# suous/RecNeXt

Measured on AMD Instinct MI355X. Metric: images/sec RecNeXt-M3 224x224 bf16, higher is better.
Workload: dtype bf16

## Files before the change

### recnext_amd/csrc/rcx_mlp.hip

```cpp
#include "rcx_common.h"
#include "rcx_launch.h"
#include "rcx_gelu.h"

namespace rcx {
namespace mlp {

typedef float f32x16 __attribute__((ext_vector_type(16)));
typedef float f32x4q __attribute__((ext_vector_type(4)));
typedef float f32x2q __attribute__((ext_vector_type(2)));
typedef __bf16 bf16x8 __attribute__((ext_vector_type(8)));
typedef __bf16 bf16x4 __attribute__((ext_vector_type(4)));
typedef unsigned u32x4q __attribute__((ext_vector_type(4)));
typedef unsigned u32x2q __attribute__((ext_vector_type(2)));

__device__ __forceinline__ void wave_sync()
{
    __builtin_amdgcn_fence(__ATOMIC_RELEASE, "wavefront");
    __builtin_amdgcn_wave_barrier();
    __builtin_amdgcn_fence(__ATOMIC_ACQUIRE, "wavefront");
}

template <int KS1, int CT, int RD>
__device__ __forceinline__ void hidden_tile_ring(const u32x4q* Lc, const float* b1t, int lane, int h, const bf16x8 (&zb)[KS1], f32x16 (&d2)[CT])
{
    constexpr int R1 = KS1 < RD ? KS1 : RD, N2 = 2 * CT, R2 = N2 < RD ? N2 : RD;
    u32x4q ring[RD];
#pragma unroll
    for (int j = 0; j < R1; ++j) ring[j] = Lc[j * 64 + lane];
    f32x16 d1;
#pragma unroll
    for (int i = 0; i < 16; ++i) d1[i] = 0.f;
#pragma unroll
    for (int ks = 0; ks < KS1; ++ks) {
        const bf16x8 a = __builtin_bit_cast(bf16x8, ring[ks % R1]);
        if (ks + R1 < KS1) ring[ks % R1] = Lc[(ks + R1) * 64 + lane];
        d1 = __builtin_amdgcn_mfma_f32_32x32x16_bf16(a, zb[ks], d1, 0, 0, 0);
    }
#pragma unroll
    for (int f = 0; f < R2; ++f) ring[f] = Lc[(KS1 + 2 * (f % CT) + f / CT) * 64 + lane];
    bf16x8 hb[2];
    gelu_f32x2 gv[8];
#pragma unroll
    for (int g = 0; g < 4; ++g) {
        const f32x4q bb = *reinterpret_cast<const f32x4q*>(b1t + 8 * g + 4 * h);
        gv[2 * g] = gelu_f32x2{d1[4 * g] + bb.x, d1[4 * g + 1] + bb.y};
        gv[2 * g + 1] = gelu_f32x2{d1[4 * g + 2] + bb.z, d1[4 * g + 3] + bb.w};
    }
    {
        gelu_f32x2 ga[4] = {gv[0], gv[1], gv[2], gv[3]}, gb[4] = {gv[4], gv[5], gv[6], gv[7]};
        gelu2x_batch<4>(ga);
        gelu2x_batch<4>(gb);
#pragma unroll
        for (int i = 0; i < 4; ++i) { gv[i] = ga[i]; gv[4 + i] = gb[i]; }
    }
#pragma unroll
    for (int g = 0; g < 4; ++g) {
        hb[g >> 1][4 * (g & 1) + 0] = (__bf16)gv[2 * g].x; hb[g >> 1][4 * (g & 1) + 1] = (__bf16)gv[2 * g].y;
        hb[g >> 1][4 * (g & 1) + 2] = (__bf16)gv[2 * g + 1].x; hb[g >> 1][4 * (g & 1) + 3] = (__bf16)gv[2 * g + 1].y;
    }
#pragma unroll
    for (int f = 0; f < N2; ++f) {
        const bf16x8 a = __builtin_bit_cast(bf16x8, ring[f % R2]);
        if (f + R2 < N2) ring[f % R2] = Lc[(KS1 + 2 * ((f + R2) % CT) + (f + R2) / CT) * 64 + lane];
        d2[f % CT] = __builtin_amdgcn_mfma_f32_32x32x16_bf16(a, hb[f / CT], d2[f % CT], 0, 0, 0);
    }
}


template <int KS1, int HT, int CT, int NW, int WPS, bool KX, bool OX, bool STAGED>
__global__ void __launch_bounds__(64 * NW, WPS)
k_channel_mlp(const bf16_t* __restrict__ z, const bf16_t* __restrict__ xres, bf16_t* __restrict__ y, const u32x4q* __restrict__ wfrag, const float* __restrict__ bias,
              int M, int C, int ntiles)
{
    extern __shared__ __attribute__((aligned(16))) unsigned char lds_raw[];
    constexpr int NF = HT * KS1 + CT * 2 * HT;
    const u32x4q* const Lf = reinterpret_cast<const u32x4q*>(lds_raw);
    const float* const Lb1 = reinterpret_cast<const float*>(lds_raw + (size_t)NF * 1024);
    const float* const Lb2 = Lb1 + 32 * HT;
    {
        u32x4q* Lw = reinterpret_cast<u32x4q*>(lds_raw);
        for (int i = threadIdx.x; i < NF * 64; i += 64 * NW) Lw[i] = wfrag[i];
        float* Lb = reinterpret_cast<float*>(lds_raw + (size_t)NF * 1024);
        for (int i = threadIdx.x; i < 32 * (HT + CT); i += 64 * NW) Lb[i] = bias[i];
    }
    __syncthreads();
    const int wave = threadIdx.x >> 6, lane = threadIdx.x & 63, r = lane & 31, h = lane >> 5;
    const unsigned nbytes = (unsigned)M * (unsigned)C * 2u;
    const __amdgpu_buffer_rsrc_t zsrc = __builtin_amdgcn_make_buffer_rsrc((void*)z, 0, nbytes, 0x00020000);
    const __amdgpu_buffer_rsrc_t xsrc = __builtin_amdgcn_make_buffer_rsrc((void*)xres, 0, nbytes, 0x00020000);
    const __amdgpu_buffer_rsrc_t ysrc = __builtin_amdgcn_make_buffer_rsrc((void*)y, 0, nbytes, 0x00020000);
    unsigned zk[KS1], oc[CT][4];
#pragma unroll
    for (int ks = 0; ks < KS1; ++ks) zk[ks] = KX || 16 * ks + 8 * h < C ? 2u * (16 * ks + 8 * h) : 0x80000000u;
#pragma unroll
    for (int ct = 0; ct < CT; ++ct)
#pragma unroll
        for (int g = 0; g < 4; ++g) oc[ct][g] = OX || 32 * ct + 8 * g + 4 * h < C ? 2u * (32 * ct + 8 * g + 4 * h) : 0x80000000u;

    auto hidden_tile = [&](int ht, const bf16x8 (&zb)[KS1], f32x16 (&d2)[CT]) {
        hidden_tile_ring<KS1, CT, 4>(Lf + (size_t)ht * (KS1 + 2 * CT) * 64, Lb1 + 32 * ht, lane, h, zb, d2);
    };
    const int stride = gridDim.x * NW;
    int tile = blockIdx.x * NW + wave;
    if constexpr (STAGED) {
        constexpr int ZP = 32 * KS1 + 16, OP = 128 * CT + 16;
        constexpr int WREG = 32 * (ZP > OP ? ZP : OP);
        unsigned char* const Lt = lds_raw + (size_t)NF * 1024 + sizeof(float) * 32 * (HT + CT) + (size_t)wave * WREG;
        const unsigned RB = 2u * (unsigned)C;
        unsigned go[KS1], za[KS1], oa[KS1];
        bool live[KS1];
#pragma unroll
        for (int i = 0; i < KS1; ++i) {
            const unsigned o = 1024u * i + 16u * lane, t = o / RB, bb = o - t * RB;
            live[i] = o < 32u * RB;
            go[i] = live[i] ? o : 0x80000000u;
            za[i] = t * ZP + bb;
            oa[i] = t * OP + 2u * bb;
        }
        u32x4q zq[KS1];
        auto load_z = [&](int t) {
#pragma unroll
            for (int i = 0; i < KS1; ++i) zq[i] = __builtin_bit_cast(u32x4q, __builtin_amdgcn_raw_buffer_load_b128(zsrc, (int)((unsigned)t * 32u * RB + go[i]), 0, 0));
        };
        if (tile < ntiles) load_z(tile);
        for (; tile < ntiles; tile += stride) {
            const unsigned base = (unsigned)tile * 32u * RB;
#pragma unroll
            for (int i = 0; i < KS1; ++i)
                if (live[i]) *reinterpret_cast<u32x4q*>(Lt + za[i]) = zq[i];
            wave_sync();
            bf16x8 zb[KS1];
#pragma unroll
            for (int ks = 0; ks < KS1; ++ks) {
                u32x4q v = *reinterpret_cast<const u32x4q*>(Lt + r * ZP + 32 * ks + 16 * h);
                if (!KX && ks == KS1 - 1 && !(16 * ks + 8 * h < C)) v = u32x4q{0u, 0u, 0u, 0u};
                zb[ks] = __builtin_bit_cast(bf16x8, v);
            }
            wave_sync();
            if (tile + stride < ntiles) load_z(tile + stride);
            u32x4q xq[KS1];
#pragma unroll
            for (int i = 0; i < KS1; ++i) xq[i] = __builtin_bit_cast(u32x4q, __builtin_amdgcn_raw_buffer_load_b128(xsrc, (int)(base + go[i]), 0, 0));
            f32x16 d2[CT];
#pragma unroll
            for (int ct = 0; ct < CT; ++ct)
#pragma unroll
                for (int i = 0; i < 16; ++i) d2[ct][i] = 0.f;
#pragma unroll 1
            for (int ht = 0; ht < HT; ++ht) hidden_tile(ht, zb, d2);
#pragma unroll
            for (int ct = 0; ct < CT; ++ct)
#pragma unroll
                for (int g = 0; g < 4; ++g) {
                    const f32x4q bb = *reinterpret_cast<const f32x4q*>(Lb2 + 32 * ct + 8 * g + 4 * h);
                    *reinterpret_cast<f32x4q*>(Lt + r * OP + 4 * (32 * ct + 8 * g + 4 * h)) =
                        f32x4q{d2[ct][4 * g] + bb.x, d2[ct][4 * g + 1] + bb.y, d2[ct][4 * g + 2] + bb.z, d2[ct][4 * g + 3] + bb.w};
                }
            wave_sync();
#pragma unroll
            for (int i = 0; i < KS1; ++i) {
                if (!live[i]) continue;
                const f32x4q lo = *reinterpret_cast<const f32x4q*>(Lt + oa[i]), hi = *reinterpret_cast<const f32x4q*>(Lt + oa[i] + 16);
                const u32x4q xv = xq[i];
                bf16x8 o;
                o[0] = (__bf16)(lo.x + __uint_as_float(xv.x << 16)); o[1] = (__bf16)(lo.y + __uint_as_float(xv.x & 0xffff0000u));
                o[2] = (__bf16)(lo.z + __uint_as_float(xv.y << 16)); o[3] = (__bf16)(lo.w + __uint_as_float(xv.y & 0xffff0000u));
                o[4] = (__bf16)(hi.x + __uint_as_float(xv.z << 16)); o[5] = (__bf16)(hi.y + __uint_as_float(xv.z & 0xffff0000u));
                o[6] = (__bf16)(hi.z + __uint_as_float(xv.w << 16)); o[7] = (__bf16)(hi.w + __uint_as_float(xv.w & 0xffff0000u));
                __builtin_amdgcn_raw_buffer_store_b128(__builtin_bit_cast(u32x4q, o), ysrc, (int)(base + go[i]), 0, 0);
            }
            wave_sync();
        }
        return;
    }
    u32x4q zf[KS1];
    auto load_z = [&](int t) {
        const unsigned row = (unsigned)(32 * t + r) * (unsigned)C * 2u;
#pragma unroll
        for (int ks = 0; ks < KS1; ++ks) zf[ks] = __builtin_bit_cast(u32x4q, __builtin_amdgcn_raw_buffer_load_b128(zsrc, (int)(row + zk[ks]), 0, 0));
    };
    if (tile < ntiles) load_z(tile);
    for (; tile < ntiles; tile += stride) {
        const unsigned row = (unsigned)(32 * tile + r) * (unsigned)C * 2u;
        bf16x8 zb[KS1];
#pragma unroll
        for (int ks = 0; ks < KS1; ++ks) zb[ks] = __builtin_bit_cast(bf16x8, zf[ks]);
        if (tile + stride < ntiles) load_z(tile + stride);
        f32x16 d2[CT];
#pragma unroll
        for (int ct = 0; ct < CT; ++ct)
#pragma unroll
            for (int i = 0; i < 16; ++i) d2[ct][i] = 0.f;
#pragma unroll 1
        for (int ht = 0; ht < HT; ++ht) hidden_tile(ht, zb, d2);
        u32x2q xr[CT][4];
#pragma unroll
        for (int ct = 0; ct < CT; ++ct)
#pragma unroll
            for (int g = 0; g < 4; ++g) xr[ct][g] = __builtin_bit_cast(u32x2q, __builtin_amdgcn_raw_buffer_load_b64(xsrc, (int)(row + oc[ct][g]), 0, 0));
#pragma unroll
        for (int ct = 0; ct < CT; ++ct)
#pragma unroll
            for (int g = 0; g < 4; ++g) {
                const f32x4q bb = *reinterpret_cast<const f32x4q*>(Lb2 + 32 * ct + 8 * g + 4 * h);
                const unsigned x0 = xr[ct][g].x, x1 = xr[ct][g].y;
                bf16x4 o;
                o[0] = (__bf16)(d2[ct][4 * g + 0] + bb.x + __uint_as_float(x0 << 16));
                o[1] = (__bf16)(d2[ct][4 * g + 1] + bb.y + __uint_as_float(x0 & 0xffff0000u));
                o[2] = (__bf16)(d2[ct][4 * g + 2] + bb.z + __uint_as_float(x1 << 16));
                o[3] = (__bf16)(d2[ct][4 * g + 3] + bb.w + __uint_as_float(x1 & 0xffff0000u));
                __builtin_amdgcn_raw_buffer_store_b64(__builtin_bit_cast(u32x2q, o), ysrc, (int)(row + oc[ct][g]), 0, 0);
            }
    }
}


template <int KS1, int HT, int CT, int NW, int WPS, int ZH, bool ZPF>
__global__ void __launch_bounds__(64 * NW, WPS)
k_channel_mlp_stream(const bf16_t* __restrict__ z, const bf16_t* __restrict__ xres, bf16_t* __restrict__ y, const u32x4q* __restrict__ wfrag, const float* __restrict__ bias,
                     int M, int C, int nblocks)
{
    extern __shared__ __attribute__((aligned(16))) unsigned char lds_raw[];
    constexpr int NCH = KS1 + 2 * CT, NT = 64 * NW, PER = (NCH * 64 + NT - 1) / NT;
    constexpr bool RAG = NCH * 64 % NT != 0;
    u32x4q* const Lring = reinterpret_cast<u32x4q*>(lds_raw);
    float* const Lb1 = reinterpret_cast<float*>(lds_raw + (size_t)2 * NCH * 1024);
    float* const Lb2 = Lb1 + 32 * HT;
    for (int i = threadIdx.x; i < 32 * (HT + CT); i += NT) Lb1[i] = bias[i];
    const int wave = threadIdx.x >> 6, lane = threadIdx.x & 63, r = lane & 31, h = lane >> 5;
    const unsigned nbytes = (unsigned)M * (unsigned)C * 2u;
    const __amdgpu_buffer_rsrc_t zsrc = __builtin_amdgcn_make_buffer_rsrc((void*)z, 0, nbytes, 0x00020000);
    const __amdgpu_buffer_rsrc_t xsrc = __builtin_amdgcn_make_buffer_rsrc((void*)xres, 0, nbytes, 0x00020000);
    const __amdgpu_buffer_rsrc_t ysrc = __builtin_amdgcn_make_buffer_rsrc((void*)y, 0, nbytes, 0x00020000);
    static_assert(HT % 2 == 0, "the ring alternates two register sets");
    u32x4q cp[2][PER];
    auto request = [&](u32x4q (&dst)[PER], int chunk) {
#pragma unroll
        for (int i = 0; i < PER; ++i)
            if (!RAG || i + 1 < PER || threadIdx.x + i * NT < NCH * 64) dst[i] = wfrag[(size_t)chunk * NCH * 64 + threadIdx.x + i * NT];
    };
    auto deposit = [&](const u32x4q (&src)[PER], int slot) {
        u32x4q* const Ln = Lring + slot * NCH * 64;
#pragma unroll
        for (int i = 0; i < PER; ++i)
            if (!RAG || i + 1 < PER || threadIdx.x + i * NT < NCH * 64) Ln[threadIdx.x + i * NT] = src[i];
    };
    request(cp[0], 0);
    deposit(cp[0], 0);
    request(cp[1], 1 % HT);
    __syncthreads();
    static_assert(CT % 2 == 0, "output in halves of two tiles");
    static_assert(KS1 % ZH == 0, "column parts of whole k-steps");
    constexpr int RB = 32 * KS1, RBH = RB / ZH, KH = KS1 / ZH, ZP = RBH + 16, OP = 256 + 16, IMG = 32 * (ZP > OP ? ZP : OP), NH = CT / 2;
    unsigned char* const Lt = lds_raw + (size_t)2 * NCH * 1024 + sizeof(float) * 32 * (HT + CT) + (size_t)wave * IMG;
    unsigned zo[KS1], za[KS1];
#pragma unroll
    for (int i = 0; i < KS1; ++i) {
        const unsigned o = 1024u * (i % KH) + 16u * lane, t = o / RBH, bz = o % RBH;
        zo[i] = t * RB + (i / KH) * RBH + bz;
        za[i] = t * ZP + bz;
    }
    const unsigned ht_tok = lane >> 3, ht_b = 16u * (lane & 7);
    u32x4q zq[KS1];
    auto load_z = [&](int blk) {
        const unsigned base = (unsigned)(32 * (blk * NW + wave)) * (unsigned)RB;
#pragma unroll
        for (int i = 0; i < KS1; ++i) zq[i] = __builtin_bit_cast(u32x4q, __builtin_amdgcn_raw_buffer_load_b128(zsrc, (int)(base + zo[i]), 0, 0));
    };
    if (ZPF && (int)blockIdx.x < nblocks) load_z(blockIdx.x);
    for (int block = blockIdx.x; block < nblocks; block += gridDim.x) {
        const unsigned base = (unsigned)(32 * (block * NW + wave)) * (unsigned)RB;
        if constexpr (!ZPF) load_z(block);
        bf16x8 zb[KS1];
#pragma unroll
        for (int q = 0; q < ZH; ++q) {
#pragma unroll
            for (int i = 0; i < KH; ++i) *reinterpret_cast<u32x4q*>(Lt + za[q * KH + i]) = zq[q * KH + i];
            wave_sync();
#pragma unroll
            for (int k = 0; k < KH; ++k) zb[q * KH + k] = __builtin_bit_cast(bf16x8, *reinterpret_cast<const u32x4q*>(Lt + r * ZP + 32 * k + 16 * h));
            wave_sync();
        }
        if (ZPF && block + (int)gridDim.x < nblocks) load_z(block + gridDim.x);
        f32x16 d2[CT];
#pragma unroll
        for (int ct = 0; ct < CT; ++ct)
#pragma unroll
            for (int i = 0; i < 16; ++i) d2[ct][i] = 0.f;
        u32x4q xq[NH][4];
#pragma unroll 1
        for (int ht = 0; ht < HT; ht += 2) {
            request(cp[0], (ht + 2) % HT);
            if (ht == HT - 2) {
#pragma unroll
                for (int hf = 0; hf < NH; ++hf)
#pragma unroll
                    for (int j = 0; j < 4; ++j)
                        xq[hf][j] = __builtin_bit_cast(u32x4q, __builtin_amdgcn_raw_buffer_load_b128(xsrc, (int)(128u * hf + ht_b < RB ? base + (8u * j + ht_tok) * RB + 128u * hf + ht_b : 0x80000000u), 0, 0));
            }
            hidden_tile_ring<KS1, CT, (NW > 4 || KS1 > 16 ? 4 : 8)>(Lring, Lb1 + 32 * ht, lane, h, zb, d2);
            deposit(cp[1], 1);
            __syncthreads();
            request(cp[1], (ht + 3) % HT);
            hidden_tile_ring<KS1, CT, (NW > 4 || KS1 > 16 ? 4 : 8)>(Lring + NCH * 64, Lb1 + 32 * (ht + 1), lane, h, zb, d2);
            deposit(cp[0], 0);
            __syncthreads();
        }
#pragma unroll
        for (int hf = 0; hf < NH; ++hf) {
#pragma unroll
            for (int c2 = 0; c2 < 2; ++c2)
#pragma unroll
                for (int g = 0; g < 4; ++g) {
                    const int ct = 2 * hf + c2;
                    const f32x4q bb = *reinterpret_cast<const f32x4q*>(Lb2 + 32 * ct + 8 * g + 4 * h);
                    *reinterpret_cast<f32x4q*>(Lt + r * OP + 4 * (32 * c2 + 8 * g + 4 * h)) =
                        f32x4q{d2[ct][4 * g] + bb.x, d2[ct][4 * g + 1] + bb.y, d2[ct][4 * g + 2] + bb.z, d2[ct][4 * g + 3] + bb.w};
                }
            wave_sync();
#pragma unroll
            for (int j = 0; j < 4; ++j) {
                const unsigned char* src = Lt + (8 * j + ht_tok) * OP + 2 * ht_b;
                const f32x4q lo = *reinterpret_cast<const f32x4q*>(src), hi = *reinterpret_cast<const f32x4q*>(src + 16);
                const u32x4q xv = xq[hf][j];
                bf16x8 o;
                o[0] = (__bf16)(lo.x + __uint_as_float(xv.x << 16)); o[1] = (__bf16)(lo.y + __uint_as_float(xv.x & 0xffff0000u));
                o[2] = (__bf16)(lo.z + __uint_as_float(xv.y << 16)); o[3] = (__bf16)(lo.w + __uint_as_float(xv.y & 0xffff0000u));
                o[4] = (__bf16)(hi.x + __uint_as_float(xv.z << 16)); o[5] = (__bf16)(hi.y + __uint_as_float(xv.z & 0xffff0000u));
                o[6] = (__bf16)(hi.z + __uint_as_float(xv.w << 16)); o[7] = (__bf16)(hi.w + __uint_as_float(xv.w & 0xffff0000u));
                __builtin_amdgcn_raw_buffer_store_b128(__builtin_bit_cast(u32x4q, o), ysrc, (int)(128u * hf + ht_b < RB ? base + (8u * j + ht_tok) * RB + 128u * hf + ht_b : 0x80000000u), 0, 0);
            }
            wave_sync();
        }
    }
}


template <int KS1, int HT, int CT>
__global__ void __launch_bounds__(512, 2)
k_channel_mlp_pair(const bf16_t* __restrict__ z, const bf16_t* __restrict__ xres, bf16_t* __restrict__ y, const u32x4q* __restrict__ wfrag, const float* __restrict__ bias,
                   int M, int C, int nblocks)
{
    extern __shared__ __attribute__((aligned(16))) unsigned char lds_raw[];
    constexpr int NW = 8, NT = 64 * NW, NS = 3, NCH = KS1 + 2 * CT, PER = NCH * 64 / NT;
    static_assert(NCH * 64 % NT == 0 && HT >= 2, "whole pieces per wave");
    constexpr int ZH = 4, RB = 32 * KS1, RBH = RB / ZH, KH = KS1 / ZH, ZP = RBH + 16, OP = 128 + 16, IMG = 32 * (ZP > OP ? ZP : OP);
    static_assert(KS1 % ZH == 0 && RBH == 128, "column parts of 64 channels: a request = 8 token rows of 128 bytes");
    u32x4q* const Lring = reinterpret_cast<u32x4q*>(lds_raw);
    float* const Lb1 = reinterpret_cast<float*>(lds_raw + (size_t)NS * NCH * 1024);
    const float* const Lb2 = Lb1 + 32 * HT;
    const int wave = threadIdx.x >> 6, lane = threadIdx.x & 63, r = lane & 31, h = lane >> 5;
    const int wv = __builtin_amdgcn_readfirstlane(wave);
    unsigned char* const Lt = lds_raw + (size_t)NS * NCH * 1024 + sizeof(float) * 32 * (HT + CT) + (size_t)wv * IMG;
    auto fill = [&](int chunk, int slot) {
        const u32x4q* src = wfrag + (size_t)chunk * NCH * 64 + threadIdx.x;
        u32x4q* dst = Lring + (size_t)slot * NCH * 64 + wv * 64;
#pragma unroll
        for (int i = 0; i < PER; ++i)
            __builtin_amdgcn_global_load_lds((__attribute__((address_space(1))) void*)(src + i * NT), (__attribute__((address_space(3))) void*)(dst + i * NT), 16, 0, 0);
    };
    constexpr int VM_ALL = 0x70, VM_NEXT = 0x70 | (PER & 15) | ((PER >> 4) << 14);
    fill(0, 0);
    fill(1, 1);
    for (int i = threadIdx.x; i < 32 * (HT + CT); i += NT) Lb1[i] = bias[i];
    const unsigned nbytes = (unsigned)M * (unsigned)C * 2u;
    const __amdgpu_buffer_rsrc_t zsrc = __builtin_amdgcn_make_buffer_rsrc((void*)z, 0, nbytes, 0x00020000);
    const __amdgpu_buffer_rsrc_t xsrc = __builtin_amdgcn_make_buffer_rsrc((void*)xres, 0, nbytes, 0x00020000);
    const __amdgpu_buffer_rsrc_t ysrc = __builtin_amdgcn_make_buffer_rsrc((void*)y, 0, nbytes, 0x00020000);
    const unsigned zo0 = (unsigned)(lane >> 3) * RB + 16u * (lane & 7), za0 = (unsigned)(lane >> 3) * ZP + 16u * (lane & 7);
    const unsigned ot = lane >> 2, ob = 16u * (lane & 3);
    if (!(__builtin_popcount(wv) & 1)) __builtin_amdgcn_s_setprio(1);
    int slot = 0;
    for (int block = blockIdx.x; block < nblocks; block += gridDim.x) {
        const unsigned base = (unsigned)(32 * (block * NW + wave)) * (unsigned)RB;
        const bool more = block + (int)gridDim.x < nblocks;
        bf16x8 zb[KS1];
        {
            u32x4q zq[KS1];
#pragma unroll
            for (int i = 0; i < KS1; ++i)
                zq[i] = __builtin_bit_cast(u32x4q, __builtin_amdgcn_raw_buffer_load_b128(zsrc, (int)(base + zo0 + 8u * RB * (i % KH) + RBH * (i / KH)), 0, 0));
#pragma unroll
            for (int q = 0; q < ZH; ++q) {
#pragma unroll
                for (int i = 0; i < KH; ++i) *reinterpret_cast<u32x4q*>(Lt + za0 + 8 * ZP * i) = zq[q * KH + i];
                wave_sync();
#pragma unroll
                for (int k = 0; k < KH; ++k) zb[q * KH + k] = __builtin_bit_cast(bf16x8, *reinterpret_cast<const u32x4q*>(Lt + r * ZP + 32 * k + 16 * h));
                wave_sync();
            }
        }
        f32x16 d2[CT];
#pragma unroll
        for (int ct = 0; ct < CT; ++ct)
#pragma unroll
            for (int i = 0; i < 16; ++i) d2[ct][i] = 0.f;
#pragma unroll 1
        for (int ht = 0; ht < HT; ++ht) {
            if (ht + 1 < HT || more) __builtin_amdgcn_s_waitcnt(VM_NEXT);
            else __builtin_amdgcn_s_waitcnt(VM_ALL);
            __builtin_amdgcn_s_barrier();
            if (ht + 2 < HT || more) fill((ht + 2) % HT, slot == 0 ? 2 : slot - 1);
            hidden_tile_ring<KS1, CT, 4>(Lring + (size_t)slot * NCH * 64, Lb1 + 32 * ht, lane, h, zb, d2);
            slot = slot == NS - 1 ? 0 : slot + 1;
        }
        u32x4q xq[CT][2];
#pragma unroll
        for (int ct = 0; ct < CT; ++ct)
#pragma unroll
            for (int j = 0; j < 2; ++j)
                xq[ct][j] = __builtin_bit_cast(u32x4q, __builtin_amdgcn_raw_buffer_load_b128(xsrc, (int)(base + (16u * j + ot) * RB + 64u * ct + ob), 0, 0));
#pragma unroll
        for (int ct = 0; ct < CT; ++ct) {
#pragma unroll
            for (int g = 0; g < 4; ++g) {
                const f32x4q bb = *reinterpret_cast<const f32x4q*>(Lb2 + 32 * ct + 8 * g + 4 * h);
                *reinterpret_cast<f32x4q*>(Lt + r * OP + 4 * (8 * g + 4 * h)) =
                    f32x4q{d2[ct][4 * g] + bb.x, d2[ct][4 * g + 1] + bb.y, d2[ct][4 * g + 2] + bb.z, d2[ct][4 * g + 3] + bb.w};
            }
            wave_sync();
#pragma unroll
            for (int j = 0; j < 2; ++j) {
                const unsigned char* src = Lt + (16 * j + ot) * OP + 2 * ob;
                const f32x4q lo = *reinterpret_cast<const f32x4q*>(src), hi = *reinterpret_cast<const f32x4q*>(src + 16);
                const u32x4q xv = xq[ct][j];
                bf16x8 o;
                o[0] = (__bf16)(lo.x + __uint_as_float(xv.x << 16)); o[1] = (__bf16)(lo.y + __uint_as_float(xv.x & 0xffff0000u));
                o[2] = (__bf16)(lo.z + __uint_as_float(xv.y << 16)); o[3] = (__bf16)(lo.w + __uint_as_float(xv.y & 0xffff0000u));
                o[4] = (__bf16)(hi.x + __uint_as_float(xv.z << 16)); o[5] = (__bf16)(hi.y + __uint_as_float(xv.z & 0xffff0000u));
                o[6] = (__bf16)(hi.z + __uint_as_float(xv.w << 16)); o[7] = (__bf16)(hi.w + __uint_as_float(xv.w & 0xffff0000u));
                __builtin_amdgcn_raw_buffer_store_b128(__builtin_bit_cast(u32x4q, o), ysrc, (int)(base + (16u * j + ot) * RB + 64u * ct + ob), 0, 0);
            }
            wave_sync();
        }
    }
}

}

static bool mlp_shape(int C, int H, int* ks1, int* ht, int* ct)
{
    if (C <= 0 || H <= 0 || C % 8 || H % 32) return false;
    *ks1 = (C + 15) / 16; *ht = H / 32; *ct = (C + 31) / 32;
    if (C > 128 && (*ct & 1)) ++*ct;
    return true;
}

bool channel_mlp_applicable(int M, int C, int H, int dtype)
{
    int ks1, ht, ct;
    if (dtype != 1 || M <= 0 || !mlp_shape(C, H, &ks1, &ht, &ct)) return false;
    if ((unsigned long long)M * C * 2 >= (1ull << 31)) return false;
    if (C == 256 && ht == 16) return true;
    if (C == 192 && ht == 12) return true;
    if ((C == 160 && ht == 10) || (C == 320 && ht == 20)) return true;
    return (ks1 == 4 && ht == 4 && ct == 2) || (C == 128 && ht == 8) || (ks1 == 3 && ht == 3 && ct == 2) || (C == 96 && ht == 6) || (C == 80 && ht == 5);
}

size_t channel_mlp_pack_bytes(int C, int H)
{
    int ks1, ht, ct;
    if (!mlp_shape(C, H, &ks1, &ht, &ct)) return 0;
    return (size_t)(ht * ks1 + ct * 2 * ht) * 1024;
}

template <int KS1, int HT, int CT, bool KX, bool OX>
static hipError_t launch_mlp(const void* z, const void* x, void* y, const void* wfrag, const float* bias, int M, int C, int ncu, hipStream_t s)
{
    constexpr size_t lds = (size_t)(HT * KS1 + CT * 2 * HT) * 1024 + sizeof(float) * 32 * (HT + CT);
    static_assert(lds <= 160 * 1024, "the weights must fit the LDS");
    constexpr int NW = CT <= 2 ? 12 : 8, WPS = NW / 4;
    constexpr bool STAGED = CT <= 2;
    constexpr size_t stage = STAGED ? (size_t)NW * 32 * ((32 * KS1 + 16) > (128 * CT + 16) ? (32 * KS1 + 16) : (128 * CT + 16)) : 0;
    if ((C == 16 * KS1) != KX || (C == 32 * CT) != OX) return hipErrorInvalidConfiguration;
    auto kfn = mlp::k_channel_mlp<KS1, HT, CT, NW, WPS, KX, OX, STAGED>;
    static_assert(lds + stage <= 160 * 1024, "weights + the waves' images must fit the LDS");
    RCX_SET_LDS_ONCE(kfn, lds + stage);
    const int ntiles = (M + 31) / 32;
    int grid = ncu;
    if (grid * NW > ntiles) grid = (ntiles + NW - 1) / NW;
    hipLaunchKernelGGL(kfn, dim3((unsigned)grid), dim3(64 * NW), lds + stage, s, (const bf16_t*)z, (const bf16_t*)x, (bf16_t*)y, (const mlp::u32x4q*)wfrag, bias, M, C, ntiles);
    return hipGetLastError();
}

template <int KS1, int HT, int CT, int NW, int ZH = 1, bool ZPF = true>
static hipError_t launch_mlp_stream(const void* z, const void* x, void* y, const void* wfrag, const float* bias, int M, int C, int ncu, hipStream_t s)
{
    constexpr int NCH = KS1 + 2 * CT, ZP = 32 * KS1 / ZH + 16, OP = 256 + 16, IMG = 32 * (ZP > OP ? ZP : OP);
    constexpr size_t lds = (size_t)2 * NCH * 1024 + sizeof(float) * 32 * (HT + CT) + (size_t)NW * IMG;
    static_assert(lds <= 160 * 1024, "the ring and the waves' images must fit the LDS");
    static_assert(CT % 2 == 0 && 32 * CT >= 16 * KS1 && 32 * (CT - 2) < 16 * KS1, "output tiles: the channel count rounded up to a multiple of 64");
    if (C != 16 * KS1) return hipErrorInvalidConfiguration;
    auto kfn = mlp::k_channel_mlp_stream<KS1, HT, CT, NW, NW / 4, ZH, ZPF>;
    RCX_SET_LDS_ONCE(kfn, lds);
    const int nblocks = (M + 32 * NW - 1) / (32 * NW);
    const int grid = nblocks < ncu ? nblocks : ncu;
    hipLaunchKernelGGL(kfn, dim3((unsigned)grid), dim3(64 * NW), lds, s, (const bf16_t*)z, (const bf16_t*)x, (bf16_t*)y, (const mlp::u32x4q*)wfrag, bias, M, C, nblocks);
    return hipGetLastError();
}

static hipError_t launch_mlp_pair256(const void* z, const void* x, void* y, const void* wfrag, const float* bias, int M, int C, int ncu, hipStream_t s)
{
    constexpr int KS1 = 16, HT = 16, CT = 8, NCH = KS1 + 2 * CT, IMG = 32 * (128 + 16);
    constexpr size_t lds = (size_t)3 * NCH * 1024 + sizeof(float) * 32 * (HT + CT) + (size_t)8 * IMG;
    static_assert(lds <= 160 * 1024, "the ring and the waves' images must fit the LDS");
    if (C != 16 * KS1) return hipErrorInvalidConfiguration;
    auto kfn = mlp::k_channel_mlp_pair<KS1, HT, CT>;
    RCX_SET_LDS_ONCE(kfn, lds);
    const int nblocks = (M + 255) / 256;
    const int grid = nblocks < ncu ? nblocks : ncu;
    hipLaunchKernelGGL(kfn, dim3((unsigned)grid), dim3(512), lds, s, (const bf16_t*)z, (const bf16_t*)x, (bf16_t*)y, (const mlp::u32x4q*)wfrag, bias, M, C, nblocks);
    return hipGetLastError();
}

hipError_t channel_mlp(const void* z, const void* x, void* y, const void* wfrag, const float* bias, int M, int C, int H, int dtype, hipStream_t s)
{
    int ks1, ht, ct;
    if (!channel_mlp_applicable(M, C, H, dtype) || !mlp_shape(C, H, &ks1, &ht, &ct)) return hipErrorInvalidConfiguration;
    static std::atomic<int> cus[RCX_MAX_DEVICES];
    int dev = 0, ncu = 256;
    if (hipGetDevice(&dev) == hipSuccess && dev >= 0 && dev < RCX_MAX_DEVICES) {
        ncu = cus[dev].load(std::memory_order_relaxed);
        if (ncu <= 0) {
            int v = 0;
            ncu = hipDeviceGetAttribute(&v, hipDeviceAttributeMultiprocessorCount, dev) == hipSuccess && v > 0 ? v : 256;
            cus[dev].store(ncu, std::memory_order_relaxed);
        }
    }
    if (C == 256 && ht == 16) return launch_mlp_pair256(z, x, y, wfrag, bias, M, C, ncu, s);
    if (C == 192 && ht == 12) return launch_mlp_stream<12, 12, 6, 4>(z, x, y, wfrag, bias, M, C, ncu, s);
    if (C == 160 && ht == 10) return launch_mlp_stream<10, 10, 6, 4>(z, x, y, wfrag, bias, M, C, ncu, s);
    if (C == 320 && ht == 20) return launch_mlp_stream<20, 20, 10, 4, 2, false>(z, x, y, wfrag, bias, M, C, ncu, s);
    if (ks1 == 4 && ht == 4) return C == 64 ? launch_mlp<4, 4, 2, true, true>(z, x, y, wfrag, bias, M, C, ncu, s)
                                            : launch_mlp<4, 4, 2, false, false>(z, x, y, wfrag, bias, M, C, ncu, s);
    if (ks1 == 8 && ht == 8) {
        if (C != 128) return hipErrorInvalidConfiguration;
        return launch_mlp_stream<8, 8, 4, 8>(z, x, y, wfrag, bias, M, C, ncu, s);
    }
    if (ks1 == 3 && ht == 3) return C == 48 ? launch_mlp<3, 3, 2, true, false>(z, x, y, wfrag, bias, M, C, ncu, s)
                                            : launch_mlp<3, 3, 2, false, false>(z, x, y, wfrag, bias, M, C, ncu, s);
    if (ks1 == 6 && ht == 6) return C == 96 ? launch_mlp<6, 6, 3, true, true>(z, x, y, wfrag, bias, M, C, ncu, s) : hipErrorInvalidConfiguration;
    if (ks1 == 5 && ht == 5) return C == 80 ? launch_mlp<5, 5, 3, true, false>(z, x, y, wfrag, bias, M, C, ncu, s) : hipErrorInvalidConfiguration;
    return hipErrorInvalidConfiguration;
}

}
```

### recnext_amd/csrc/rcx_opts.h

```cpp
#pragma once
#include <stdlib.h>
#include <mutex>
#include <string>

namespace rcx {
namespace opt {

enum Id { FORCE_GENERIC, CPL, CPL14, CPL14_RL, CPT, CPT_CB, CPT16, UPADD_CPL, UPADD_CPT, NESTED, TRAIN_FUSED, BWD_FUSED, WGRAD_CPL, COUNT };

namespace detail {
inline const char* name_of(int i)
{
    static const char* const k[COUNT] = {"RCX_FORCE_GENERIC", "RCX_CPL", "RCX_CPL14", "RCX_CPL14_RL", "RCX_CPT", "RCX_CPT_CB", "RCX_CPT16",
                                         "RCX_UPADD_CPL", "RCX_UPADD_CPT", "RCX_NESTED", "RCX_TRAIN_FUSED", "RCX_BWD_FUSED", "RCX_WGRAD_CPL"};
    return k[i];
}
struct Table {
    std::string val[COUNT];
    std::once_flag once;
    void read()
    {
        for (int i = 0; i < COUNT; ++i) {
            const char* v = getenv(name_of(i));
            val[i] = v ? v : "";
        }
    }
};
inline Table& table() { static Table t; return t; }
}

inline const char* str(Id id)
{
    detail::Table& t = detail::table();
    std::call_once(t.once, [&] { t.read(); });
    return t.val[id].c_str();
}
inline bool off(Id id) { return str(id)[0] == '0'; }
inline bool on(Id id) { const char* v = str(id); return *v && *v != '0'; }
inline int int_or(Id id, int dflt) { const char* v = str(id); return *v ? atoi(v) : dflt; }
inline void reload()
{
    detail::Table& t = detail::table();
    std::call_once(t.once, [&] { t.read(); });
    t.read();
}

inline bool hand_kernels_off() { return on(FORCE_GENERIC); }

}
}
```

Measured before the change: 117,700.

## Add free-running channel MLP kernels with per-slot LDS counters instead of block barriers

Adds two new channel-MLP kernels, selected by default unless RCX_MLP_FREE=0. For C=128 a resident-weight kernel assigns tiles per wave and reshapes z and residual data through per-wave LDS images. For C=256 a 4-slot weight ring replaces s_barrier with LDS full/done counters polled by each wave, with optional s_setprio on alternating waves. The aim is to stop waves lock-stepping on block barriers and to coalesce global loads and stores, at the cost of spin-wait polling, extra LDS round trips and more LDS use. Optional s_memtime stamp instrumentation is also added behind a compile flag.

```diff
diff --git a/recnext_amd/csrc/rcx_mlp.hip b/recnext_amd/csrc/rcx_mlp.hip
--- a/recnext_amd/csrc/rcx_mlp.hip
+++ b/recnext_amd/csrc/rcx_mlp.hip
@@ -1,6 +1,41 @@
 #include "rcx_common.h"
 #include "rcx_launch.h"
 #include "rcx_gelu.h"
+#include "rcx_opts.h"
+
+#ifdef RCX_MLP_STAMPS
+#define RCX_MLP_NST 9
+#define RCX_MLP_STAMP(k)                                                                                        \
+    {                                                                                                           \
+        __builtin_amdgcn_sched_barrier(0);                                                                      \
+        unsigned long long t_;                                                                                  \
+        asm volatile("s_memtime %0\n\ts_waitcnt lgkmcnt(0)" : "=s"(t_)::"memory");                              \
+        __builtin_amdgcn_sched_barrier(0);                                                                      \
+        tsum[k] += t_ - tlast;                                                                                  \
+        tlast = t_;                                                                                             \
+    }
+#define RCX_MLP_STAMP_PARAMS , unsigned long long (&tsum)[RCX_MLP_NST], unsigned long long& tlast
+#define RCX_MLP_STAMP_PASS , tsum, tlast
+#define RCX_MLP_STAMP_ARG , unsigned long long* __restrict__ stamps
+#define RCX_MLP_STAMP_VAL , g_mlp_stamps
+#define RCX_MLP_STAMP_BEGIN                                                                                     \
+    unsigned long long tsum[RCX_MLP_NST] = {}, tlast;                                                           \
+    asm volatile("s_memtime %0\n\ts_waitcnt lgkmcnt(0)" : "=s"(tlast)::"memory");
+#define RCX_MLP_STAMP_END                                                                                       \
+    if ((threadIdx.x & 63) == 0)                                                                                \
+        for (int k_ = 0; k_ < RCX_MLP_NST; ++k_) stamps[((size_t)blockIdx.x * 8 + (threadIdx.x >> 6)) * RCX_MLP_NST + k_] = tsum[k_];
+namespace rcx {
+static unsigned long long* g_mlp_stamps = nullptr;
+}
+#else
+#define RCX_MLP_STAMP(k)
+#define RCX_MLP_STAMP_PARAMS
+#define RCX_MLP_STAMP_PASS
+#define RCX_MLP_STAMP_ARG
+#define RCX_MLP_STAMP_VAL
+#define RCX_MLP_STAMP_BEGIN
+#define RCX_MLP_STAMP_END
+#endif
 
 namespace rcx {
 namespace mlp {
@@ -21,7 +56,7 @@
 }
 
 template <int KS1, int CT, int RD>
-__device__ __forceinline__ void hidden_tile_ring(const u32x4q* Lc, const float* b1t, int lane, int h, const bf16x8 (&zb)[KS1], f32x16 (&d2)[CT])
+__device__ __forceinline__ void hidden_tile_ring(const u32x4q* Lc, const float* b1t, int lane, int h, const bf16x8 (&zb)[KS1], f32x16 (&d2)[CT] RCX_MLP_STAMP_PARAMS)
 {
     constexpr int R1 = KS1 < RD ? KS1 : RD, N2 = 2 * CT, R2 = N2 < RD ? N2 : RD;
     u32x4q ring[RD];
@@ -30,12 +65,14 @@
     f32x16 d1;
 #pragma unroll
     for (int i = 0; i < 16; ++i) d1[i] = 0.f;
+    RCX_MLP_STAMP(2)
 #pragma unroll
     for (int ks = 0; ks < KS1; ++ks) {
         const bf16x8 a = __builtin_bit_cast(bf16x8, ring[ks % R1]);
         if (ks + R1 < KS1) ring[ks % R1] = Lc[(ks + R1) * 64 + lane];
         d1 = __builtin_amdgcn_mfma_f32_32x32x16_bf16(a, zb[ks], d1, 0, 0, 0);
     }
+    RCX_MLP_STAMP(3)
 #pragma unroll
     for (int f = 0; f < R2; ++f) ring[f] = Lc[(KS1 + 2 * (f % CT) + f / CT) * 64 + lane];
     bf16x8 hb[2];
@@ -58,12 +95,14 @@
         hb[g >> 1][4 * (g & 1) + 0] = (__bf16)gv[2 * g].x; hb[g >> 1][4 * (g & 1) + 1] = (__bf16)gv[2 * g].y;
         hb[g >> 1][4 * (g & 1) + 2] = (__bf16)gv[2 * g + 1].x; hb[g >> 1][4 * (g & 1) + 3] = (__bf16)gv[2 * g + 1].y;
     }
+    RCX_MLP_STAMP(4)
 #pragma unroll
     for (int f = 0; f < N2; ++f) {
         const bf16x8 a = __builtin_bit_cast(bf16x8, ring[f % R2]);
         if (f + R2 < N2) ring[f % R2] = Lc[(KS1 + 2 * ((f + R2) % CT) + (f + R2) / CT) * 64 + lane];
         d2[f % CT] = __builtin_amdgcn_mfma_f32_32x32x16_bf16(a, hb[f / CT], d2[f % CT], 0, 0, 0);
     }
+    RCX_MLP_STAMP(5)
 }
 
 
@@ -72,6 +111,7 @@
 k_channel_mlp(const bf16_t* __restrict__ z, const bf16_t* __restrict__ xres, bf16_t* __restrict__ y, const u32x4q* __restrict__ wfrag, const float* __restrict__ bias,
               int M, int C, int ntiles)
 {
+    RCX_MLP_STAMP_BEGIN
     extern __shared__ __attribute__((aligned(16))) unsigned char lds_raw[];
     constexpr int NF = HT * KS1 + CT * 2 * HT;
     const u32x4q* const Lf = reinterpret_cast<const u32x4q*>(lds_raw);
@@ -98,7 +138,7 @@
         for (int g = 0; g < 4; ++g) oc[ct][g] = OX || 32 * ct + 8 * g + 4 * h < C ? 2u * (32 * ct + 8 * g + 4 * h) : 0x80000000u;
 
     auto hidden_tile = [&](int ht, const bf16x8 (&zb)[KS1], f32x16 (&d2)[CT]) {
-        hidden_tile_ring<KS1, CT, 4>(Lf + (size_t)ht * (KS1 + 2 * CT) * 64, Lb1 + 32 * ht, lane, h, zb, d2);
+        hidden_tile_ring<KS1, CT, 4>(Lf + (size_t)ht * (KS1 + 2 * CT) * 64, Lb1 + 32 * ht, lane, h, zb, d2 RCX_MLP_STAMP_PASS);
     };
     const int stride = gridDim.x * NW;
     int tile = blockIdx.x * NW + wave;
@@ -220,6 +260,7 @@
 k_channel_mlp_stream(const bf16_t* __restrict__ z, const bf16_t* __restrict__ xres, bf16_t* __restrict__ y, const u32x4q* __restrict__ wfrag, const float* __restrict__ bias,
                      int M, int C, int nblocks)
 {
+    RCX_MLP_STAMP_BEGIN
     extern __shared__ __attribute__((aligned(16))) unsigned char lds_raw[];
     constexpr int NCH = KS1 + 2 * CT, NT = 64 * NW, PER = (NCH * 64 + NT - 1) / NT;
     constexpr bool RAG = NCH * 64 % NT != 0;
@@ -298,11 +339,11 @@
                     for (int j = 0; j < 4; ++j)
                         xq[hf][j] = __builtin_bit_cast(u32x4q, __builtin_amdgcn_raw_buffer_load_b128(xsrc, (int)(128u * hf + ht_b < RB ? base + (8u * j + ht_tok) * RB + 128u * hf + ht_b : 0x80000000u), 0, 0));
             }
-            hidden_tile_ring<KS1, CT, (NW > 4 || KS1 > 16 ? 4 : 8)>(Lring, Lb1 + 32 * ht, lane, h, zb, d2);
+            hidden_tile_ring<KS1, CT, (NW > 4 || KS1 > 16 ? 4 : 8)>(Lring, Lb1 + 32 * ht, lane, h, zb, d2 RCX_MLP_STAMP_PASS);
             deposit(cp[1], 1);
             __syncthreads();
             request(cp[1], (ht + 3) % HT);
-            hidden_tile_ring<KS1, CT, (NW > 4 || KS1 > 16 ? 4 : 8)>(Lring + NCH * 64, Lb1 + 32 * (ht + 1), lane, h, zb, d2);
+            hidden_tile_ring<KS1, CT, (NW > 4 || KS1 > 16 ? 4 : 8)>(Lring + NCH * 64, Lb1 + 32 * (ht + 1), lane, h, zb, d2 RCX_MLP_STAMP_PASS);
             deposit(cp[0], 0);
             __syncthreads();
         }
@@ -339,8 +380,9 @@
 template <int KS1, int HT, int CT>
 __global__ void __launch_bounds__(512, 2)
 k_channel_mlp_pair(const bf16_t* __restrict__ z, const bf16_t* __restrict__ xres, bf16_t* __restrict__ y, const u32x4q* __restrict__ wfrag, const float* __restrict__ bias,
-                   int M, int C, int nblocks)
-{
+                   int M, int C, int nblocks RCX_MLP_STAMP_ARG)
+{
+    RCX_MLP_STAMP_BEGIN
     extern __shared__ __attribute__((aligned(16))) unsigned char lds_raw[];
     constexpr int NW = 8, NT = 64 * NW, NS = 3, NCH = KS1 + 2 * CT, PER = NCH * 64 / NT;
     static_assert(NCH * 64 % NT == 0 && HT >= 2, "whole pieces per wave");
@@ -395,13 +437,19 @@
         for (int ct = 0; ct < CT; ++ct)
 #pragma unroll
             for (int i = 0; i < 16; ++i) d2[ct][i] = 0.f;
+        RCX_MLP_STAMP(6)
 #pragma unroll 1
         for (int ht = 0; ht < HT; ++ht) {
             if (ht + 1 < HT || more) __builtin_amdgcn_s_waitcnt(VM_NEXT);
             else __builtin_amdgcn_s_waitcnt(VM_ALL);
+            RCX_MLP_STAMP(0)
             __builtin_amdgcn_s_barrier();
+            RCX_MLP_STAMP(1)
+#ifdef RCX_MLP_STAMPS
+            tsum[8] += 1;
+#endif
             if (ht + 2 < HT || more) fill((ht + 2) % HT, slot == 0 ? 2 : slot - 1);
-            hidden_tile_ring<KS1, CT, 4>(Lring + (size_t)slot * NCH * 64, Lb1 + 32 * ht, lane, h, zb, d2);
+            hidden_tile_ring<KS1, CT, 4>(Lring + (size_t)slot * NCH * 64, Lb1 + 32 * ht, lane, h, zb, d2 RCX_MLP_STAMP_PASS);
             slot = slot == NS - 1 ? 0 : slot + 1;
         }
         u32x4q xq[CT][2];
@@ -433,7 +481,249 @@
             }
             wave_sync();
         }
-    }
+        RCX_MLP_STAMP(7)
+    }
+    RCX_MLP_STAMP_END
+}
+
+
+constexpr int FREE_ZP = 128 + 16, FREE_OP = 256 + 16, FREE_IMG = 16 * FREE_ZP > 8 * FREE_OP ? 16 * FREE_ZP : 8 * FREE_OP;
+
+__device__ __forceinline__ int fresh_lane()
+{
+    unsigned t = threadIdx.x;
+    asm volatile("" : "+v"(t));
+    return (int)(t & 63u);
+}
+
+template <int KS1>
+__device__ __forceinline__ void free_z_requests(u32x4q (&zq)[KS1], __amdgpu_buffer_rsrc_t zsrc, unsigned base)
+{
+    constexpr int NZ = KS1 / 4, RB = 32 * KS1;
+    const int lane = fresh_lane();
+    const unsigned off = base + (unsigned)(lane >> 3) * RB + 16u * (lane & 7);
+#pragma unroll
+    for (int i = 0; i < KS1; ++i)
+        zq[i] = __builtin_bit_cast(u32x4q, __builtin_amdgcn_raw_buffer_load_b128(zsrc, (int)(off + (16u * (i / (2 * NZ)) + 8u * (i % 2)) * RB + 128u * ((i / 2) % NZ)), 0, 0));
+}
+
+template <int KS1>
+__device__ __forceinline__ void free_z_fragments(const u32x4q (&zq)[KS1], bf16x8 (&zb)[KS1], unsigned char* Lt)
+{
+    constexpr int NZ = KS1 / 4;
+    const int lane = fresh_lane(), r = lane & 31, h = lane >> 5;
+    unsigned char* const wr = Lt + (lane >> 3) * FREE_ZP + 16 * (lane & 7);
+    const unsigned char* const rd = Lt + (r & 15) * FREE_ZP + 16 * h;
+#pragma unroll
+    for (int p = 0; p < 2; ++p)
+#pragma unroll
+        for (int q = 0; q < NZ; ++q) {
+#pragma unroll
+            for (int j = 0; j < 2; ++j) *reinterpret_cast<u32x4q*>(wr + 8 * FREE_ZP * j) = zq[(p * NZ + q) * 2 + j];
+            wave_sync();
+#pragma unroll
+            for (int k = 0; k < 4; ++k) {
+                const u32x4q v = *reinterpret_cast<const u32x4q*>(rd + 32 * k);
+                zb[4 * q + k] = __builtin_bit_cast(bf16x8, p == 0 || r >= 16 ? v : __builtin_bit_cast(u32x4q, zb[4 * q + k]));
+            }
+            wave_sync();
+        }
+}
+
+template <int CT>
+__device__ __forceinline__ void free_x_requests(u32x4q (&xq)[2 * CT], __amdgpu_buffer_rsrc_t xsrc, unsigned base)
+{
+    constexpr int RB = 64 * CT;
+    const int lane = fresh_lane();
+    const unsigned off = base + (unsigned)(lane >> 3) * RB + 16u * (lane & 7);
+#pragma unroll
+    for (int i = 0; i < 2 * CT; ++i)
+        xq[i] = __builtin_bit_cast(u32x4q, __builtin_amdgcn_raw_buffer_load_b128(xsrc, (int)(off + 8u * RB * (i % 4) + 128u * (i / 4)), 0, 0));
+}
+
+template <int CT>
+__device__ __forceinline__ void free_y_rows(const f32x16 (&d2)[CT], const u32x4q (&xq)[2 * CT], const float* Lb2, unsigned char* Lt, __amdgpu_buffer_rsrc_t ysrc, unsigned base)
+{
+    constexpr int NH = CT / 2, RB = 64 * CT;
+    const int lane = fresh_lane(), r = lane & 31, h = lane >> 5;
+    const unsigned off = base + (unsigned)(lane >> 3) * RB + 16u * (lane & 7);
+    unsigned char* const wr = Lt + (r & 7) * FREE_OP + 16 * h;
+    const unsigned char* const rd = Lt + (lane >> 3) * FREE_OP + 32 * (lane & 7);
+#pragma unroll
+    for (int hf = 0; hf < NH; ++hf)
+#pragma unroll
+        for (int p4 = 0; p4 < 4; ++p4) {
+            if ((r >> 3) == p4) {
+#pragma unroll
+                for (int c2 = 0; c2 < 2; ++c2)
+#pragma unroll
+                    for (int g = 0; g < 4; ++g) {
+                        const int ct = 2 * hf + c2;
+                        const f32x4q bb = *reinterpret_cast<const f32x4q*>(Lb2 + 32 * ct + 8 * g + 4 * h);
+                        *reinterpret_cast<f32x4q*>(wr + 4 * (32 * c2 + 8 * g)) =
+                            f32x4q{d2[ct][4 * g] + bb.x, d2[ct][4 * g + 1] + bb.y, d2[ct][4 * g + 2] + bb.z, d2[ct][4 * g + 3] + bb.w};
+                    }
+            }
+            wave_sync();
+            const f32x4q lo = *reinterpret_cast<const f32x4q*>(rd), hi = *reinterpret_cast<const f32x4q*>(rd + 16);
+            const u32x4q xv = xq[4 * hf + p4];
+            bf16x8 o;
+            o[0] = (__bf16)(lo.x + __uint_as_float(xv.x << 16)); o[1] = (__bf16)(lo.y + __uint_as_float(xv.x & 0xffff0000u));
+            o[2] = (__bf16)(lo.z + __uint_as_float(xv.y << 16)); o[3] = (__bf16)(lo.w + __uint_as_float(xv.y & 0xffff0000u));
+            o[4] = (__bf16)(hi.x + __uint_as_float(xv.z << 16)); o[5] = (__bf16)(hi.y + __uint_as_float(xv.z & 0xffff0000u));
+            o[6] = (__bf16)(hi.z + __uint_as_float(xv.w << 16)); o[7] = (__bf16)(hi.w + __uint_as_float(xv.w & 0xffff0000u));
+            __builtin_amdgcn_raw_buffer_store_b128(__builtin_bit_cast(u32x4q, o), ysrc, (int)(off + 8u * RB * p4 + 128u * hf), 0, 0);
+            wave_sync();
+        }
+}
+
+template <int KS1, int HT, int CT>
+__global__ void __launch_bounds__(512, 2)
+k_channel_mlp_free(const bf16_t* __restrict__ z, const bf16_t* __restrict__ xres, bf16_t* __restrict__ y, const u32x4q* __restrict__ wfrag, const float* __restrict__ bias,
+                   int M, int C, int ntiles)
+{
+    RCX_MLP_STAMP_BEGIN
+    extern __shared__ __attribute__((aligned(16))) unsigned char lds_raw[];
+    constexpr int NW = 8, NT = 64 * NW, NCH = KS1 + 2 * CT, NF = HT * NCH, RB = 32 * KS1;
+    static_assert(KS1 % 4 == 0 && CT % 2 == 0 && 32 * CT == 16 * KS1, "whole 64-channel parts, no padding lanes");
+    const u32x4q* const Lf = reinterpret_cast<const u32x4q*>(lds_raw);
+    const float* const Lb1 = reinterpret_cast<const float*>(lds_raw + (size_t)NF * 1024);
+    const float* const Lb2 = Lb1 + 32 * HT;
+    const int lane = threadIdx.x & 63, h = lane >> 5;
+    const int wv = __builtin_amdgcn_readfirstlane(threadIdx.x >> 6);
+    unsigned char* const Lt = lds_raw + (size_t)NF * 1024 + sizeof(float) * 32 * (HT + CT) + (size_t)wv * FREE_IMG;
+    const unsigned nbytes = (unsigned)M * (unsigned)C * 2u;
+    const __amdgpu_buffer_rsrc_t zsrc = __builtin_amdgcn_make_buffer_rsrc((void*)z, 0, nbytes, 0x00020000);
+    const __amdgpu_buffer_rsrc_t xsrc = __builtin_amdgcn_make_buffer_rsrc((void*)xres, 0, nbytes, 0x00020000);
+    const __amdgpu_buffer_rsrc_t ysrc = __builtin_amdgcn_make_buffer_rsrc((void*)y, 0, nbytes, 0x00020000);
+    const int stride = gridDim.x * NW;
+    int tile = wv * (int)gridDim.x + (int)blockIdx.x;
+    u32x4q zq[KS1];
+    if (tile < ntiles) free_z_requests<KS1>(zq, zsrc, (unsigned)tile * 32u * RB);
+    {
+        u32x4q* Lw = reinterpret_cast<u32x4q*>(lds_raw);
+        for (int i = threadIdx.x; i < NF * 64; i += NT) Lw[i] = wfrag[i];
+        float* Lb = reinterpret_cast<float*>(lds_raw + (size_t)NF * 1024);
+        for (int i = threadIdx.x; i < 32 * (HT + CT); i += NT) Lb[i] = bias[i];
+    }
+    __syncthreads();
+    for (; tile < ntiles; tile += stride) {
+        const unsigned off = (unsigned)tile * 32u * RB;
+        bf16x8 zb[KS1];
+        free_z_fragments<KS1>(zq, zb, Lt);
+        if (tile + stride < ntiles) free_z_requests<KS1>(zq, zsrc, (unsigned)(tile + stride) * 32u * RB);
+        f32x16 d2[CT];
+#pragma unroll
+        for (int ct = 0; ct < CT; ++ct)
+#pragma unroll
+            for (int i = 0; i < 16; ++i) d2[ct][i] = 0.f;
+        u32x4q xq[2 * CT];
+#pragma unroll 1
+        for (int ht = 0; ht < HT; ++ht) {
+            if (ht == HT - 2) free_x_requests<CT>(xq, xsrc, off);
+            hidden_tile_ring<KS1, CT, 4>(Lf + (size_t)ht * NCH * 64, Lb1 + 32 * ht, lane, h, zb, d2 RCX_MLP_STAMP_PASS);
+        }
+        free_y_rows<CT>(d2, xq, Lb2, Lt, ysrc, off);
+    }
+}
+
+__device__ __forceinline__ unsigned lds_addr(const void* p)
+{
+    return (unsigned)(__UINTPTR_TYPE__)(__attribute__((address_space(3))) const void*)p;
+}
+__device__ __forceinline__ void lds_add_one(unsigned addr)
+{
+    if ((threadIdx.x & 63) == 0) asm volatile("ds_add_u32 %0, %1" ::"v"(addr), "v"(1u) : "memory");
+}
+__device__ __forceinline__ void lds_wait_ge(unsigned addr, unsigned target)
+{
+    for (;;) {
+        unsigned v;
+        asm volatile("ds_read_b32 %0, %1\n\ts_waitcnt lgkmcnt(0)" : "=v"(v) : "v"(addr) : "memory");
+        if (__builtin_amdgcn_readfirstlane(v) >= target) break;
+        __builtin_amdgcn_s_sleep(1);
+    }
+}
+
+template <int KS1, int HT, int CT, bool PRIO>
+__global__ void __launch_bounds__(512, 2)
+k_channel_mlp_pair_free(const bf16_t* __restrict__ z, const bf16_t* __restrict__ xres, bf16_t* __restrict__ y, const u32x4q* __restrict__ wfrag, const float* __restrict__ bias,
+                        int M, int C, int nblocks RCX_MLP_STAMP_ARG)
+{
+    RCX_MLP_STAMP_BEGIN
+    extern __shared__ __attribute__((aligned(16))) unsigned char lds_raw[];
+    constexpr int NW = 8, NT = 64 * NW, NS = 4, NCH = KS1 + 2 * CT, PER = NCH * 64 / NT, RB = 32 * KS1;
+    static_assert(NCH * 64 % NT == 0 && HT >= 2, "whole pieces per wave");
+    static_assert(KS1 % 4 == 0 && CT % 2 == 0 && 32 * CT == 16 * KS1, "whole 64-channel parts, no padding lanes");
+    u32x4q* const Lring = reinterpret_cast<u32x4q*>(lds_raw);
+    float* const Lb1 = reinterpret_cast<float*>(lds_raw + (size_t)NS * NCH * 1024);
+    const float* const Lb2 = Lb1 + 32 * HT;
+    unsigned* const Lfull = reinterpret_cast<unsigned*>(Lb1 + 32 * (HT + CT));
+    const unsigned full0 = __builtin_amdgcn_readfirstlane(lds_addr(Lfull)), done0 = full0 + 4u * NS;
+    const int lane = threadIdx.x & 63, h = lane >> 5;
+    const int wv = __builtin_amdgcn_readfirstlane(threadIdx.x >> 6);
+    unsigned char* const Lt = lds_raw + (size_t)NS * NCH * 1024 + sizeof(float) * 32 * (HT + CT) + 64 + (size_t)wv * FREE_IMG;
+    auto fill = [&](int chunk, int slot) {
+        unsigned t = threadIdx.x;
+        asm volatile("" : "+v"(t));
+        const u32x4q* src = wfrag + (size_t)chunk * NCH * 64 + t;
+        u32x4q* dst = Lring + (size_t)slot * NCH * 64 + wv * 64;
+#pragma unroll
+        for (int i = 0; i < PER; ++i)
+            __builtin_amdgcn_global_load_lds((__attribute__((address_space(1))) void*)(src + i * NT), (__attribute__((address_space(3))) void*)(dst + i * NT), 16, 0, 0);
+    };
+    static_assert(PER < 16, "vmcnt(PER) as an assembler immediate");
+    fill(0, 0);
+    fill(1, 1);
+    for (int i = threadIdx.x; i < 32 * (HT + CT); i += NT) Lb1[i] = bias[i];
+    if (threadIdx.x < 2 * NS) Lfull[threadIdx.x] = 0u;
+    asm volatile("s_waitcnt lgkmcnt(0)\n\ts_barrier" ::: "memory");
+    const unsigned nbytes = (unsigned)M * (unsigned)C * 2u;
+    const __amdgpu_buffer_rsrc_t zsrc = __builtin_amdgcn_make_buffer_rsrc((void*)z, 0, nbytes, 0x00020000);
+    const __amdgpu_buffer_rsrc_t xsrc = __builtin_amdgcn_make_buffer_rsrc((void*)xres, 0, nbytes, 0x00020000);
+    const __amdgpu_buffer_rsrc_t ysrc = __builtin_amdgcn_make_buffer_rsrc((void*)y, 0, nbytes, 0x00020000);
+    if (PRIO && !(__builtin_popcount(wv) & 1)) __builtin_amdgcn_s_setprio(1);
+    unsigned g = 0;
+    for (int block = blockIdx.x; block < nblocks; block += gridDim.x) {
+        const unsigned off = (unsigned)(32 * (block * NW + wv)) * (unsigned)RB;
+        const bool more = block + (int)gridDim.x < nblocks;
+        bf16x8 zb[KS1];
+        {
+            u32x4q zq[KS1];
+            free_z_requests<KS1>(zq, zsrc, off);
+            free_z_fragments<KS1>(zq, zb, Lt);
+        }
+        f32x16 d2[CT];
+#pragma unroll
+        for (int ct = 0; ct < CT; ++ct)
+#pragma unroll
+            for (int i = 0; i < 16; ++i) d2[ct][i] = 0.f;
+        RCX_MLP_STAMP(6)
+#pragma unroll 1
+        for (int ht = 0; ht < HT; ++ht, ++g) {
+            const unsigned slot = g % NS;
+            if (ht + 1 < HT || more) asm volatile("s_waitcnt vmcnt(%0)" ::"n"(PER) : "memory");
+            else asm volatile("s_waitcnt vmcnt(0)" ::: "memory");
+            RCX_MLP_STAMP(0)
+            lds_add_one(full0 + 4u * slot);
+            lds_wait_ge(full0 + 4u * slot, NW * (g / NS + 1));
+            RCX_MLP_STAMP(1)
+#ifdef RCX_MLP_STAMPS
+            tsum[8] += 1;
+#endif
+            if (ht + 2 < HT || more) {
+                lds_wait_ge(done0 + 4u * ((g + 2) % NS), NW * ((g + 2) / NS));
+                fill((ht + 2) % HT, (g + 2) % NS);
+            }
+            hidden_tile_ring<KS1, CT, 4>(Lring + (size_t)slot * NCH * 64, Lb1 + 32 * ht, lane, h, zb, d2 RCX_MLP_STAMP_PASS);
+            lds_add_one(done0 + 4u * slot);
+        }
+        u32x4q xq[2 * CT];
+        free_x_requests<CT>(xq, xsrc, off);
+        free_y_rows<CT>(d2, xq, Lb2, Lt, ysrc, off);
+        RCX_MLP_STAMP(7)
+    }
+    RCX_MLP_STAMP_END
 }
 
 }
@@ -509,7 +799,36 @@
     RCX_SET_LDS_ONCE(kfn, lds);
     const int nblocks = (M + 255) / 256;
     const int grid = nblocks < ncu ? nblocks : ncu;
-    hipLaunchKernelGGL(kfn, dim3((unsigned)grid), dim3(512), lds, s, (const bf16_t*)z, (const bf16_t*)x, (bf16_t*)y, (const mlp::u32x4q*)wfrag, bias, M, C, nblocks);
+    hipLaunchKernelGGL(kfn, dim3((unsigned)grid), dim3(512), lds, s, (const bf16_t*)z, (const bf16_t*)x, (bf16_t*)y, (const mlp::u32x4q*)wfrag, bias, M, C, nblocks RCX_MLP_STAMP_VAL);
+    return hipGetLastError();
+}
+
+static hipError_t launch_mlp_free128(const void* z, const void* x, void* y, const void* wfrag, const float* bias, int M, int C, int ncu, hipStream_t s)
+{
+    constexpr int KS1 = 8, HT = 8, CT = 4, NW = 8;
+    constexpr size_t lds = (size_t)HT * (KS1 + 2 * CT) * 1024 + sizeof(float) * 32 * (HT + CT) + (size_t)NW * mlp::FREE_IMG;
+    static_assert(lds <= 160 * 1024, "the pack and the waves' images must fit the LDS");
+    if (C != 16 * KS1) return hipErrorInvalidConfiguration;
+    auto kfn = mlp::k_channel_mlp_free<KS1, HT, CT>;
+    RCX_SET_LDS_ONCE(kfn, lds);
+    const int ntiles = (M + 31) / 32, nblocks = (ntiles + NW - 1) / NW;
+    const int grid = nblocks < ncu ? nblocks : ncu;
+    hipLaunchKernelGGL(kfn, dim3((unsigned)grid), dim3(64 * NW), lds, s, (const bf16_t*)z, (const bf16_t*)x, (bf16_t*)y, (const mlp::u32x4q*)wfrag, bias, M, C, ntiles);
+    return hipGetLastError();
+}
+
+template <bool PRIO>
+static hipError_t launch_mlp_pair256_free(const void* z, const void* x, void* y, const void* wfrag, const float* bias, int M, int C, int ncu, hipStream_t s)
+{
+    constexpr int KS1 = 16, HT = 16, CT = 8, NCH = KS1 + 2 * CT;
+    constexpr size_t lds = (size_t)4 * NCH * 1024 + sizeof(float) * 32 * (HT + CT) + 64 + (size_t)8 * mlp::FREE_IMG;
+    static_assert(lds <= 160 * 1024, "the ring and the waves' images must fit the LDS");
+    if (C != 16 * KS1) return hipErrorInvalidConfiguration;
+    auto kfn = mlp::k_channel_mlp_pair_free<KS1, HT, CT, PRIO>;
+    RCX_SET_LDS_ONCE(kfn, lds);
+    const int nblocks = (M + 255) / 256;
+    const int grid = nblocks < ncu ? nblocks : ncu;
+    hipLaunchKernelGGL(kfn, dim3((unsigned)grid), dim3(512), lds, s, (const bf16_t*)z, (const bf16_t*)x, (bf16_t*)y, (const mlp::u32x4q*)wfrag, bias, M, C, nblocks RCX_MLP_STAMP_VAL);
     return hipGetLastError();
 }
 
@@ -527,7 +846,11 @@
             cus[dev].store(ncu, std::memory_order_relaxed);
         }
     }
-    if (C == 256 && ht == 16) return launch_mlp_pair256(z, x, y, wfrag, bias, M, C, ncu, s);
+    const bool lockstep = opt::off(opt::MLP_FREE);
+    if (C == 256 && ht == 16) {
+        if (lockstep) return launch_mlp_pair256(z, x, y, wfrag, bias, M, C, ncu, s);
+        return opt::str(opt::MLP_FREE)[0] == 'n' ? launch_mlp_pair256_free<false>(z, x, y, wfrag, bias, M, C, ncu, s) : launch_mlp_pair256_free<true>(z, x, y, wfrag, bias, M, C, ncu, s);
+    }
     if (C == 192 && ht == 12) return launch_mlp_stream<12, 12, 6, 4>(z, x, y, wfrag, bias, M, C, ncu, s);
     if (C == 160 && ht == 10) return launch_mlp_stream<10, 10, 6, 4>(z, x, y, wfrag, bias, M, C, ncu, s);
     if (C == 320 && ht == 20) return launch_mlp_stream<20, 20, 10, 4, 2, false>(z, x, y, wfrag, bias, M, C, ncu, s);
@@ -535,7 +858,7 @@
                                             : launch_mlp<4, 4, 2, false, false>(z, x, y, wfrag, bias, M, C, ncu, s);
     if (ks1 == 8 && ht == 8) {
         if (C != 128) return hipErrorInvalidConfiguration;
-        return launch_mlp_stream<8, 8, 4, 8>(z, x, y, wfrag, bias, M, C, ncu, s);
+        return lockstep ? launch_mlp_stream<8, 8, 4, 8>(z, x, y, wfrag, bias, M, C, ncu, s) : launch_mlp_free128(z, x, y, wfrag, bias, M, C, ncu, s);
     }
     if (ks1 == 3 && ht == 3) return C == 48 ? launch_mlp<3, 3, 2, true, false>(z, x, y, wfrag, bias, M, C, ncu, s)
                                             : launch_mlp<3, 3, 2, false, false>(z, x, y, wfrag, bias, M, C, ncu, s);
@@ -545,3 +868,12 @@
 }
 
 }
+
+#ifdef RCX_MLP_STAMPS
+extern "C" int rcx_mlp_diag_fwd(const void* z, const void* x, void* y, const void* wfrag, const float* bias, int M, int C, int H, void* stamps, void* stream)
+{
+    rcx::g_mlp_stamps = (unsigned long long*)stamps;
+    rcx::opt::reload();
+    return (int)rcx::channel_mlp(z, x, y, wfrag, bias, M, C, H, 1, (hipStream_t)stream);
+}
+#endif
diff --git a/recnext_amd/csrc/rcx_opts.h b/recnext_amd/csrc/rcx_opts.h
--- a/recnext_amd/csrc/rcx_opts.h
+++ b/recnext_amd/csrc/rcx_opts.h
@@ -6,13 +6,13 @@
 namespace rcx {
 namespace opt {
 
-enum Id { FORCE_GENERIC, CPL, CPL14, CPL14_RL, CPT, CPT_CB, CPT16, UPADD_CPL, UPADD_CPT, NESTED, TRAIN_FUSED, BWD_FUSED, WGRAD_CPL, COUNT };
+enum Id { FORCE_GENERIC, CPL, CPL14, CPL14_RL, CPT, CPT_CB, CPT16, UPADD_CPL, UPADD_CPT, NESTED, TRAIN_FUSED, BWD_FUSED, WGRAD_CPL, MLP_FREE, COUNT };
 
 namespace detail {
 inline const char* name_of(int i)
 {
     static const char* const k[COUNT] = {"RCX_FORCE_GENERIC", "RCX_CPL", "RCX_CPL14", "RCX_CPL14_RL", "RCX_CPT", "RCX_CPT_CB", "RCX_CPT16",
-                                         "RCX_UPADD_CPL", "RCX_UPADD_CPT", "RCX_NESTED", "RCX_TRAIN_FUSED", "RCX_BWD_FUSED", "RCX_WGRAD_CPL"};
+                                         "RCX_UPADD_CPL", "RCX_UPADD_CPT", "RCX_NESTED", "RCX_TRAIN_FUSED", "RCX_BWD_FUSED", "RCX_WGRAD_CPL", "RCX_MLP_FREE"};
     return k[i];
 }
 struct Table {
```

New measurement: 111,900. 0.951x the previous value.
